# hby1320/pytorch_object_detection

Hardware: AMD Instinct MI355X
Metric: images/sec HISFCOS-R50 640x640 inference (higher is better)
Workload: dtype f32

## Files before the change

### include/fcosdet.h

```cpp
#ifndef FCOSDET_H_
#define FCOSDET_H_

#include <stdint.h>

#ifdef __cplusplus
extern "C" {
#endif

#define FD_OK 0
#define FD_E_INVAL (-1)
#define FD_E_UNSUPPORTED (-2)
#define FD_E_LAUNCH (-3)

#define FD_MAX_SEG 8

#define FD_ACT_NONE 0
#define FD_ACT_RELU 1
#define FD_ACT_SILU 2
#define FD_ACT_EXP 3
#define FD_ACT_SIGMOID 4

typedef void* fd_stream_t;

typedef struct fd_segs {
// ... 33 lines not shown
#define FD_TILE_WINOGRAD4 16
#define FD_TILE_NARROW 17
#define FD_TILE_F16K64 18
#define FD_TILE_COUNT 19

typedef struct fd_conv_params {
    const float* x;
    const float* w;
    const float* scale;
    const float* shift;
    const float* res;
    float* y;
    int32_t x_cs, x_co;
    int32_t res_cs, res_co;
    int32_t y_cs, y_co;
    int32_t Cin, Cout, KH, KW, stride, pad, dil;
    int32_t act;
    int32_t act_c0;
    int32_t mode;
    int32_t tile;
    int32_t tag;
    int32_t ksplit;
    void* workspace;
    int64_t workspace_bytes;
    int32_t precision;
    int32_t res_mode;
    float seg_param[FD_MAX_SEG];
    fd_segs in;
    int32_t out_H, out_W;
    int32_t sc_sy, sc_sx, sc_oy, sc_ox, sc_H, sc_W;
    const float* gate;
    int32_t gate_cs;
    int32_t reserved0;
    const float* w_frag;
    float* gn_stats;
    int32_t gn_groups;
    int32_t gate_act;
    const float* gate_b;
    const float* x2;
    int32_t x2_cs, x2_co, x2_Cin, x2_stride, x2_H, x2_W;
    int32_t wg_first, wg_count;
    int32_t sk_wgs;
    int32_t io_f16;
} fd_conv_params;
int64_t fd_conv_sk_workspace_bytes(int32_t sk_wgs);

int32_t fd_conv2d_nhwc_f32(const fd_conv_params* p, fd_stream_t stream);
int32_t fd_conv_workgroups(const fd_conv_params* p);
int32_t fd_conv_workgroups_live(const fd_conv_params* p);
typedef struct fd_b2b_params {
    const float* x; const float* w1_frag; const float* scale1; const float* shift1; const float* res; float* y;
    const float* w2_frag; const float* scale2; const float* shift2; float* z;
    int32_t x_cs, x_co, res_cs, res_co, y_cs, y_co, z_cs, z_co;
    int32_t K1, N1, N2, act1, act2, reserved0;
    int64_t rows;
} fd_b2b_params;
int32_t fd_conv1x1_b2b_f32(const fd_b2b_params* p, fd_stream_t stream);
int32_t fd_conv_narrow_nco(int32_t Cout);
int64_t fd_conv_workspace_bytes(int64_t out_rows, int32_t Cout, int32_t ksplit);

int64_t fd_wino4_weight_bytes(int32_t N, int32_t K);
int32_t fd_wino4_pack_weights_f32(const float* w, const float* scale, float* out, int32_t Cout, int32_t Cin, int32_t mode, fd_stream_t stream);

int64_t fd_conv_weight_wave_bytes(int32_t Cout, int32_t Cin);
int32_t fd_pack_conv_weight_wave_f32(const float* w, float* out, int32_t Cout, int32_t Cin, fd_stream_t stream);

int64_t fd_wino_weight_bytes(int32_t Cout, int32_t Cin);
int32_t fd_wino_pack_weights_f32(const float* w, const float* scale, float* out, int32_t Cout, int32_t Cin, int32_t mode,
                                 fd_stream_t stream);

typedef struct fd_conv_wgrad_params {
    const float* x;
    const float* dy;
    float* dw;
    int32_t x_cs, x_co, dy_cs, dy_co;
    int32_t Cin, Cout, KH, KW, stride, pad, dil;
    void* workspace;
    int64_t workspace_bytes;
    int32_t nsplit;
    int32_t layout;
    const float* scale;
    fd_segs in;
    int32_t precision;
    int32_t io_f16;
} fd_conv_wgrad_params;

int64_t fd_conv_wgrad_workspace_bytes(int64_t out_rows, int32_t Cin, int32_t Cout, int32_t KH, int32_t KW);
int32_t fd_conv2d_bwd_weight_f32(const fd_conv_wgrad_params* p, fd_stream_t stream);
int32_t fd_pack_conv_weight_f32(const float* w, const float* scale, float* out, int32_t Cout, int32_t Cin, int32_t KH,
                                int32_t KW, int32_t mode, fd_stream_t stream);

typedef struct fd_pack_job {
    const float* w;
    const float* scale;
    float* out;
    int32_t Cout, Cin, KH, KW, mode, reserved;
} fd_pack_job;
int32_t fd_pack_conv_weights_batch_f32(const fd_pack_job* jobs_dev, int32_t n_jobs, int64_t max_elems, fd_stream_t stream);

int32_t fd_stem7x7_nhwc4(const float* x4, const float* w, const float* scale, const float* shift, float* y, int32_t y_cs, int32_t y_co,
                         int32_t N, int32_t H, int32_t W, int32_t act, fd_stream_t stream);

int32_t fd_stem7x7_pool_nhwc4(const float* x4, const float* w, const float* scale, const float* shift, float* y_pooled, int32_t y_cs, int32_t y_co,
                              int32_t N, int32_t H, int32_t W, fd_stream_t stream);

int32_t fd_stem7x7_nchw3(const float* x, const float* w, const float* scale, const float* shift, float* y, int32_t y_cs, int32_t y_co,
                         int32_t N, int32_t H, int32_t W, int32_t act, int32_t pool, fd_stream_t stream);

// ... 214 lines not shown
```

### pytorch_object_detection_amd/_lib.py

```python
from __future__ import annotations

import ctypes as C
import os

FD_MAX_SEG = 8
ACT_NONE, ACT_RELU, ACT_SILU, ACT_EXP, ACT_SIGMOID = 0, 1, 2, 3, 4
CONV_GENERIC, CONV_STEM = 0, 1
PREC_F32, PREC_F16X3, PREC_F16 = 0, 1, 2
TILES = {1: (128, 128), 2: (128, 64), 3: (64, 128), 4: (64, 64), 5: (128, 32), 6: (128, 96),
         7: (128, 128), 8: (128, 64), 9: (64, 128),
         10: (256, 128), 11: (256, 128),
         12: (128, 96),
         13: (128, 128),
         15: (64, 64)}
PATCH_TILE = 13
WAVE_TILE = 15
WINO_TILE = 14
WINO4_TILE = 16
NARROW_TILE = 17
F16K64_TILE = 18

_HERE = os.path.dirname(os.path.abspath(__file__))
LIB_PATH = os.environ.get("FD_LIB") or os.path.join(_HERE, "csrc", "libfcosdet_hip.so")


class FdError(RuntimeError):

    def __init__(self, msg: str = "", rc=None):
        super().__init__(msg)
        self.rc = rc


E_INVAL, E_UNSUPPORTED, E_LAUNCH = -1, -2, -3


class Segs(C.Structure):
    _fields_ = [("nseg", C.c_int32), ("batch", C.c_int32), ("H", C.c_int32 * FD_MAX_SEG), ("W", C.c_int32 * FD_MAX_SEG),
                ("m_start", C.c_int32 * (FD_MAX_SEG + 1))]

    @staticmethod
    def make(batch: int, hw) -> "Segs":
        s = Segs()
        s.nseg, s.batch = len(hw), batch
        m = 0
        for i, (h, w) in enumerate(hw):
            s.H[i], s.W[i], s.m_start[i] = h, w, m
            m += batch * h * w
        for i in range(len(hw), FD_MAX_SEG + 1):
            s.m_start[i] = m
        return s

    @property
    def rows(self) -> int:
        return self.m_start[self.nseg]

    def level_hw(self):
        return [(self.H[i], self.W[i]) for i in range(self.nseg)]


class B2BParams(C.Structure):
    _fields_ = [("x", C.c_void_p), ("w1_frag", C.c_void_p), ("scale1", C.c_void_p), ("shift1", C.c_void_p), ("res", C.c_void_p), ("y", C.c_void_p),
                ("w2_frag", C.c_void_p), ("scale2", C.c_void_p), ("shift2", C.c_void_p), ("z", C.c_void_p),
                ("x_cs", C.c_int32), ("x_co", C.c_int32), ("res_cs", C.c_int32), ("res_co", C.c_int32), ("y_cs", C.c_int32), ("y_co", C.c_int32),
                ("z_cs", C.c_int32), ("z_co", C.c_int32),
                ("K1", C.c_int32), ("N1", C.c_int32), ("N2", C.c_int32), ("act1", C.c_int32), ("act2", C.c_int32), ("reserved0", C.c_int32),
                ("rows", C.c_int64)]


class ConvParams(C.Structure):
    _fields_ = [("x", C.c_void_p), ("w", C.c_void_p), ("scale", C.c_void_p), ("shift", C.c_void_p), ("res", C.c_void_p),
                ("y", C.c_void_p),
                ("x_cs", C.c_int32), ("x_co", C.c_int32), ("res_cs", C.c_int32), ("res_co", C.c_int32),
                ("y_cs", C.c_int32), ("y_co", C.c_int32),
                ("Cin", C.c_int32), ("Cout", C.c_int32), ("KH", C.c_int32), ("KW", C.c_int32), ("stride", C.c_int32),
                ("pad", C.c_int32), ("dil", C.c_int32),
                ("act", C.c_int32), ("act_c0", C.c_int32), ("mode", C.c_int32), ("tile", C.c_int32), ("tag", C.c_int32), ("ksplit", C.c_int32),
                ("workspace", C.c_void_p), ("workspace_bytes", C.c_int64), ("precision", C.c_int32), ("res_mode", C.c_int32),
                ("seg_param", C.c_float * FD_MAX_SEG), ("segs", Segs),
                ("out_H", C.c_int32), ("out_W", C.c_int32), ("sc_sy", C.c_int32), ("sc_sx", C.c_int32), ("sc_oy", C.c_int32),
                ("sc_ox", C.c_int32), ("sc_H", C.c_int32), ("sc_W", C.c_int32),
                ("gate", C.c_void_p), ("gate_cs", C.c_int32), ("reserved0", C.c_int32), ("w_frag", C.c_void_p),
                ("gn_stats", C.c_void_p), ("gn_groups", C.c_int32), ("gate_act", C.c_int32), ("gate_b", C.c_void_p),
                ("x2", C.c_void_p), ("x2_cs", C.c_int32), ("x2_co", C.c_int32), ("x2_Cin", C.c_int32), ("x2_stride", C.c_int32), ("x2_H", C.c_int32),
                ("x2_W", C.c_int32), ("wg_first", C.c_int32), ("wg_count", C.c_int32), ("sk_wgs", C.c_int32), ("io_f16", C.c_int32)]


class PackJob(C.Structure):
    _fields_ = [("w", C.c_void_p), ("scale", C.c_void_p), ("out", C.c_void_p), ("Cout", C.c_int32), ("Cin", C.c_int32),
                ("KH", C.c_int32), ("KW", C.c_int32), ("mode", C.c_int32), ("reserved", C.c_int32)]


class WgradParams(C.Structure):
    _fields_ = [("x", C.c_void_p), ("dy", C.c_void_p), ("dw", C.c_void_p),
                ("x_cs", C.c_int32), ("x_co", C.c_int32), ("dy_cs", C.c_int32), ("dy_co", C.c_int32),
                ("Cin", C.c_int32), ("Cout", C.c_int32), ("KH", C.c_int32), ("KW", C.c_int32), ("stride", C.c_int32),
                ("pad", C.c_int32), ("dil", C.c_int32),
                ("workspace", C.c_void_p), ("workspace_bytes", C.c_int64), ("nsplit", C.c_int32), ("layout", C.c_int32),
                ("scale", C.c_void_p), ("segs", Segs), ("precision", C.c_int32), ("io_f16", C.c_int32)]


_lib = None

_P, _I, _F, _D, _L = C.c_void_p, C.c_int32, C.c_float, C.c_double, C.c_int64
_SIGS = {
    "fd_version": (_I, []),
    "fd_last_error": (C.c_char_p, []),
    "fd_conv2d_nhwc_f32": (_I, [C.POINTER(ConvParams), _P]),
    "fd_conv_narrow_nco": (_I, [_I]),
    "fd_conv_workgroups": (_I, [C.POINTER(ConvParams)]),
    "fd_conv_workgroups_live": (_I, [C.POINTER(ConvParams)]),
    "fd_conv1x1_b2b_f32": (_I, [C.POINTER(B2BParams), _P]),
    "fd_conv_workspace_bytes": (_L, [_L, _I, _I]),
    "fd_conv_sk_workspace_bytes": (_L, [_I]),
    "fd_mbconv_pool_bytes": (_L, [_I, _I, _I, _I, _I, _I]),
    "fd_mbconv_expand_dw_nhwc": (_I, [_P, _I, _I, _P, _P, _P, _P, _P, _P, _P, _I, _I, _P, _I, _I, _I, _I, _I, _I, _I, _I, _I, _I, _I, _P]),
    "fd_se_gate_from_pool": (_I, [_P, _I, _P, _P, _P, _P, _I, _I, _I, _I, _P, _P]),
    "fd_conv_wgrad_workspace_bytes": (_L, [_L, _I, _I, _I, _I]),
    "fd_pack_conv_weight_f32": (_I, [_P, _P, _P, _I, _I, _I, _I, _I, _P]),
    "fd_pack_conv_weights_batch_f32": (_I, [_P, _I, _L, _P]),
# ... 100 lines not shown
```

### pytorch_object_detection_amd/csrc/fd_conv_b2b.hip

```cpp
#include "fd_conv_common.h"

struct B2BArgs {
    const float* x; const float* res; float* y; float* z;
    const float* scale1; const float* shift1; const float* scale2; const float* shift2;
    int x_cs, x_co, res_cs, res_co, y_cs, y_co, z_cs, z_co;
    int M, KT1, NT1, N2, act1, act2;
    unsigned x_bytes, y_bytes, z_bytes, res_bytes;
};

template <int TM, int TN2>
__global__ __launch_bounds__(64, 2) void conv1x1_b2b_kernel(B2BArgs a, const float* __restrict__ wf1_, const float* __restrict__ wf2_) {
    extern __shared__ __attribute__((aligned(16))) char smem[];
    float* As = reinterpret_cast<float*>(smem);
    float* A2 = As + 32 * TM * 32;
    constexpr int NL = 4 * TM;
    const int lane = threadIdx.x, l31 = lane & 31, lh = lane >> 5;
    const int m0 = blockIdx.x * 32 * TM;

    constexpr unsigned OOB = 0xC0000000u;
    const __amdgpu_buffer_rsrc_t xrsrc = __builtin_amdgcn_make_buffer_rsrc((void*)a.x, (short)0, (int)a.x_bytes, 0x00020000);
    const int lrow = lane >> 3, chunk = lane & 7;
    unsigned a_off[NL];
#pragma unroll
    for (int i = 0; i < NL; ++i) {
        const int m = m0 + lrow + 8 * i;
        a_off[i] = (m < a.M) ? ((unsigned)m * (unsigned)a.x_cs + (unsigned)(a.x_co + chunk * 4)) * 4u : OOB;
    }
    const float4* __restrict__ wf1 = reinterpret_cast<const float4*>(wf1_) + lane;
    const float4* __restrict__ wf2 = reinterpret_cast<const float4*>(wf2_) + lane;
    const int KT1 = a.KT1, KT2 = 2 * a.NT1;

    float4 ra[NL];
    auto load_a = [&](int kt) {
        const unsigned kb = (unsigned)kt * 128u;
#pragma unroll
        for (int i = 0; i < NL; ++i)
            ra[i] = __builtin_bit_cast(float4, __builtin_amdgcn_raw_buffer_load_b128(xrsrc, (int)(a_off[i] + kb), 0, 0));
    };
    auto store_a = [&]() {
#pragma unroll
        for (int i = 0; i < NL; ++i) *reinterpret_cast<float4*>(As + lds_off(lrow + 8 * i, chunk)) = ra[i];
    };

    f32x16 acc2[TM][TN2];
#pragma unroll
    for (int i = 0; i < TM; ++i)
#pragma unroll
        for (int j = 0; j < TN2; ++j)
#pragma unroll
            for (int e = 0; e < 16; ++e) acc2[i][j][e] = 0.f;

    const int c4 = (lane & 7) * 4, prow = lane >> 3;
    float* stage = As;
    const __amdgpu_buffer_rsrc_t yrsrc = __builtin_amdgcn_make_buffer_rsrc((void*)a.y, (short)0, (int)a.y_bytes, 0x00020000);
    const __amdgpu_buffer_rsrc_t zrsrc = __builtin_amdgcn_make_buffer_rsrc((void*)a.z, (short)0, (int)a.z_bytes, 0x00020000);
    const __amdgpu_buffer_rsrc_t rrsrc = __builtin_amdgcn_make_buffer_rsrc((void*)(a.res ? a.res : a.x), (short)0, (int)a.res_bytes, 0x00020000);
    const unsigned y_off = ((unsigned)(m0 + prow) * (unsigned)a.y_cs + (unsigned)(a.y_co + c4)) * 4u;
    const unsigned z_off = ((unsigned)(m0 + prow) * (unsigned)a.z_cs + (unsigned)(a.z_co + c4)) * 4u;
    const unsigned r_off = ((unsigned)(m0 + prow) * (unsigned)a.res_cs + (unsigned)(a.res_co + c4)) * 4u;

    for (int n1t = 0; n1t < a.NT1; ++n1t) {
        f32x16 acc1[TM][2];
#pragma unroll
        for (int i = 0; i < TM; ++i)
#pragma unroll
            for (int j = 0; j < 2; ++j)
#pragma unroll
                for (int e = 0; e < 16; ++e) acc1[i][j][e] = 0.f;
        float4 fb[2][2];
        const float4* __restrict__ w1t = wf1 + (size_t)n1t * KT1 * 512;
        load_a(0);
#pragma unroll
        for (int j = 0; j < 2; ++j)
#pragma unroll
            for (int s = 0; s < 2; ++s) fb[j][s] = w1t[(j * 4 + s) * 64];
        for (int kt = 0; kt < KT1; ++kt) {
            store_a();
            __builtin_amdgcn_sched_barrier(0);
            if (kt + 1 < KT1) load_a(kt + 1);
            __builtin_amdgcn_sched_barrier(0);
            wave_lds_sync();
            const float4* __restrict__ wc_ = w1t + (size_t)kt * 512;
            const float4* __restrict__ wn_ = w1t + (size_t)min(kt + 1, KT1 - 1) * 512;
            __builtin_amdgcn_s_setprio(1);
#pragma unroll
            for (int s = 0; s < 4; ++s) {
                float4 fa[TM];
#pragma unroll
                for (int i = 0; i < TM; ++i) fa[i] = *reinterpret_cast<const float4*>(As + lds_off(i * 32 + l31, 2 * s + lh));
#pragma unroll
                for (int i = 0; i < TM; ++i)
#pragma unroll
                    for (int j = 0; j < 2; ++j) {
                        acc1[i][j] = __builtin_amdgcn_mfma_f32_32x32x2f32(fa[i].x, fb[j][s & 1].x, acc1[i][j], 0, 0, 0);
                        acc1[i][j] = __builtin_amdgcn_mfma_f32_32x32x2f32(fa[i].y, fb[j][s & 1].y, acc1[i][j], 0, 0, 0);
                        acc1[i][j] = __builtin_amdgcn_mfma_f32_32x32x2f32(fa[i].z, fb[j][s & 1].z, acc1[i][j], 0, 0, 0);
                        acc1[i][j] = __builtin_amdgcn_mfma_f32_32x32x2f32(fa[i].w, fb[j][s & 1].w, acc1[i][j], 0, 0, 0);
                    }
#pragma unroll
                for (int j = 0; j < 2; ++j) fb[j][s & 1] = s < 2 ? wc_[(j * 4 + s + 2) * 64] : wn_[(j * 4 + s - 2) * 64];
                __builtin_amdgcn_sched_barrier(0);
            }
            __builtin_amdgcn_s_setprio(0);
            wave_lds_sync();
        }

#pragma unroll
        for (int j = 0; j < 2; ++j) {
            const int nb = n1t * 64 + 32 * j;
            const float sc = a.scale1 ? a.scale1[nb + l31] : 1.0f, sf = a.shift1 ? a.shift1[nb + l31] : 0.0f;
            float4 fb2[TN2][2];
            const int kt2 = 2 * n1t + j;
            auto w2at = [&](int jj, int s) { return wf2[((size_t)((jj >> 1) * KT2 + kt2) * 8 + (jj & 1) * 4 + s) * 64]; };
#pragma unroll
            for (int jj = 0; jj < TN2; ++jj)
#pragma unroll
                for (int s = 0; s < 2; ++s) fb2[jj][s] = w2at(jj, s);
#pragma unroll
            for (int i = 0; i < TM; ++i) {
                float4 rr[4];
#pragma unroll
                for (int p = 0; p < 4; ++p)
                    rr[p] = __builtin_bit_cast(float4, __builtin_amdgcn_raw_buffer_load_b128(rrsrc, (int)r_off, ((32 * i + 8 * p) * a.res_cs + nb) * 4, 0));
#pragma unroll
                for (int e = 0; e < 16; ++e) stage[((e & 3) + 8 * (e >> 2) + 4 * lh) * 32 + l31] = acc1[i][j][e] * sc + sf;
                wave_lds_sync();
#pragma unroll
                for (int p = 0; p < 4; ++p) {
                    float4 v = *reinterpret_cast<const float4*>(stage + (prow + 8 * p) * 32 + c4);
                    const float4 r = rr[p];
                    v.x += r.x; v.y += r.y; v.z += r.z; v.w += r.w;
                    if (a.act1 == FD_ACT_RELU) {
                        v.x = fmaxf(v.x, 0.f); v.y = fmaxf(v.y, 0.f); v.z = fmaxf(v.z, 0.f); v.w = fmaxf(v.w, 0.f);
                    } else if (a.act1 == FD_ACT_SILU) {
                        v.x = fd_act(v.x, FD_ACT_SILU, 0.f); v.y = fd_act(v.y, FD_ACT_SILU, 0.f); v.z = fd_act(v.z, FD_ACT_SILU, 0.f); v.w = fd_act(v.w, FD_ACT_SILU, 0.f);
                    }
                    __builtin_amdgcn_raw_buffer_store_b128(__builtin_bit_cast(f32x4, v), yrsrc, (int)y_off, ((32 * i + 8 * p) * a.y_cs + nb) * 4, 0);
                    *reinterpret_cast<float4*>(A2 + lds_off(32 * i + prow + 8 * p, lane & 7)) = v;
                }
                wave_lds_sync();
            }
            __builtin_amdgcn_s_setprio(1);
#pragma unroll
            for (int s = 0; s < 4; ++s) {
                float4 fa[TM];
#pragma unroll
                for (int i = 0; i < TM; ++i) fa[i] = *reinterpret_cast<const float4*>(A2 + lds_off(i * 32 + l31, 2 * s + lh));
#pragma unroll
                for (int i = 0; i < TM; ++i)
#pragma unroll
                    for (int jj = 0; jj < TN2; ++jj) {
                        acc2[i][jj] = __builtin_amdgcn_mfma_f32_32x32x2f32(fa[i].x, fb2[jj][s & 1].x, acc2[i][jj], 0, 0, 0);
                        acc2[i][jj] = __builtin_amdgcn_mfma_f32_32x32x2f32(fa[i].y, fb2[jj][s & 1].y, acc2[i][jj], 0, 0, 0);
                        acc2[i][jj] = __builtin_amdgcn_mfma_f32_32x32x2f32(fa[i].z, fb2[jj][s & 1].z, acc2[i][jj], 0, 0, 0);
                        acc2[i][jj] = __builtin_amdgcn_mfma_f32_32x32x2f32(fa[i].w, fb2[jj][s & 1].w, acc2[i][jj], 0, 0, 0);
                    }
                if (s < 2) {
#pragma unroll
                    for (int jj = 0; jj < TN2; ++jj) fb2[jj][s & 1] = w2at(jj, s + 2);
                }
                __builtin_amdgcn_sched_barrier(0);
            }
            __builtin_amdgcn_s_setprio(0);
            wave_lds_sync();
        }
    }

#pragma unroll
    for (int jj = 0; jj < TN2; ++jj) {
        const int nb = 32 * jj;
        if (nb >= a.N2) break;
        const float sc = a.scale2 ? a.scale2[nb + l31] : 1.0f, sf = a.shift2 ? a.shift2[nb + l31] : 0.0f;
#pragma unroll
        for (int i = 0; i < TM; ++i) {
#pragma unroll
            for (int e = 0; e < 16; ++e) stage[((e & 3) + 8 * (e >> 2) + 4 * lh) * 32 + l31] = acc2[i][jj][e] * sc + sf;
            wave_lds_sync();
#pragma unroll
            for (int p = 0; p < 4; ++p) {
                float4 v = *reinterpret_cast<const float4*>(stage + (prow + 8 * p) * 32 + c4);
                if (a.act2 == FD_ACT_RELU) {
                    v.x = fmaxf(v.x, 0.f); v.y = fmaxf(v.y, 0.f); v.z = fmaxf(v.z, 0.f); v.w = fmaxf(v.w, 0.f);
                } else if (a.act2 == FD_ACT_SILU) {
                    v.x = fd_act(v.x, FD_ACT_SILU, 0.f); v.y = fd_act(v.y, FD_ACT_SILU, 0.f); v.z = fd_act(v.z, FD_ACT_SILU, 0.f); v.w = fd_act(v.w, FD_ACT_SILU, 0.f);
                }
                __builtin_amdgcn_raw_buffer_store_b128(__builtin_bit_cast(f32x4, v), zrsrc, (int)z_off, ((32 * i + 8 * p) * a.z_cs + nb) * 4, 0);
            }
            wave_lds_sync();
        }
    }
}

extern "C" int32_t fd_conv1x1_b2b_f32(const fd_b2b_params* p, fd_stream_t stream_) {
    hipStream_t stream = (hipStream_t)stream_;
    FD_REQUIRE(p && p->x && p->w1_frag && p->w2_frag && p->y && p->z, FD_E_INVAL, "fd_conv1x1_b2b: null pointer");
    FD_REQUIRE(p->rows >= 1 && p->K1 >= 32 && p->K1 % 32 == 0 && p->N1 >= 64 && p->N1 % 64 == 0 && (p->N2 == 64 || p->N2 == 128), FD_E_UNSUPPORTED,
               "fd_conv1x1_b2b: needs K1 %% 32 == 0, N1 %% 64 == 0, N2 in {64, 128} (got %d -> %d -> %d)", p->K1, p->N1, p->N2);
    FD_REQUIRE(p->x_cs % 4 == 0 && p->x_co % 4 == 0 && p->x_cs >= p->x_co + p->K1 && p->y_cs % 4 == 0 && p->y_co % 4 == 0 && p->y_cs >= p->y_co + p->N1 &&
                   p->z_cs % 4 == 0 && p->z_co % 4 == 0 && p->z_cs >= p->z_co + p->N2 &&
                   (!p->res || (p->res_cs % 4 == 0 && p->res_co % 4 == 0 && p->res_cs >= p->res_co + p->N1)),
               FD_E_INVAL, "fd_conv1x1_b2b: channel views must be 4-aligned and in range");
    FD_REQUIRE((((uintptr_t)p->x | (uintptr_t)p->y | (uintptr_t)p->z | (uintptr_t)p->res | (uintptr_t)p->w1_frag | (uintptr_t)p->w2_frag) & 15) == 0, FD_E_INVAL,
               "fd_conv1x1_b2b: pointers must be 16-byte aligned");
    auto act_ok = [](int a_) { return a_ == FD_ACT_NONE || a_ == FD_ACT_RELU || a_ == FD_ACT_SILU; };
    FD_REQUIRE(act_ok(p->act1) && act_ok(p->act2), FD_E_UNSUPPORTED, "fd_conv1x1_b2b: activations none / ReLU / SiLU");
    const long xb = (long)p->rows * p->x_cs * 4;
    FD_REQUIRE(xb < 0xC0000000L - 65536 && (long)p->rows * p->y_cs * 4 < 0xC0000000L && (long)p->rows * p->z_cs * 4 < 0xC0000000L &&
                   (!p->res || (long)p->rows * p->res_cs * 4 < 0xC0000000L), FD_E_UNSUPPORTED, "fd_conv1x1_b2b: a view's buffer exceeds 3 GiB");
    B2BArgs a;
    a.x = p->x; a.res = p->res; a.y = p->y; a.z = p->z;
    a.scale1 = p->scale1; a.shift1 = p->shift1; a.scale2 = p->scale2; a.shift2 = p->shift2;
    a.x_cs = p->x_cs; a.x_co = p->x_co; a.res_cs = p->res_cs; a.res_co = p->res_co; a.y_cs = p->y_cs; a.y_co = p->y_co; a.z_cs = p->z_cs; a.z_co = p->z_co;
    a.M = (int)p->rows; a.KT1 = p->K1 / 32; a.NT1 = p->N1 / 64; a.N2 = p->N2; a.act1 = p->act1; a.act2 = p->act2;
    a.x_bytes = (unsigned)xb;
    a.y_bytes = (unsigned)((long)p->rows * p->y_cs * 4); a.z_bytes = (unsigned)((long)p->rows * p->z_cs * 4);
    a.res_bytes = p->res ? (unsigned)((long)p->rows * p->res_cs * 4) : 0u;
    if (p->N2 == 64) {
        const unsigned blocks = (unsigned)((p->rows + 63) / 64);
        hipLaunchKernelGGL((conv1x1_b2b_kernel<2, 2>), dim3(blocks), dim3(64), 2 * 64 * 32 * 4, stream, a, p->w1_frag, p->w2_frag);
    } else {
        const unsigned blocks = (unsigned)((p->rows + 31) / 32);
        hipLaunchKernelGGL((conv1x1_b2b_kernel<1, 4>), dim3(blocks), dim3(64), 2 * 32 * 32 * 4, stream, a, p->w1_frag, p->w2_frag);
    }
    FD_CHECK_LAUNCH("fd_conv1x1_b2b_f32");
    return FD_OK;
}
```

### pytorch_object_detection_amd/engine.py

```python
from __future__ import annotations

from typing import Callable, Dict, List, Optional, Sequence, Tuple

import torch

from . import ops
from . import _lib
from ._lib import ACT_EXP, ACT_NONE, ACT_RELU, ACT_SILU, FdError, Segs
from .ops import Rows


import os as _os

CONV_PRECISION = _os.environ.get("FD_CONV_PRECISION", "f32")
AUTOTUNE = True
GN_FUSED = _os.environ.get("FD_GN_FUSED", "1") != "0"
B2B_MIN_ROWS = 64 * 1024
B2B_LAYERS = "1"


class PRows(Rows):
    __slots__ = ("_flat",)


class Pool:

    def __init__(self, device):
        self.device = device
        self.free: List[torch.Tensor] = []
        self.total = 0

    def get(self, rows: int, C: int) -> PRows:
        need = rows * C
        best = None
        for i, t in enumerate(self.free):
            if t.numel() >= need and (best is None or t.numel() < self.free[best].numel()):
                best = i
        if best is None:
            flat = torch.empty(need, dtype=torch.float32, device=self.device)
            self.total += need * 4
        else:
            flat = self.free.pop(best)
        r = PRows(flat[:need].view(rows, C))
        r._flat = flat
        return r

    def put(self, r: PRows) -> None:
        self.free.append(r._flat)


class Plan:
    def __init__(self, device, precision: Optional[str] = None, pair_tuned: bool = False):
        self.device = device
        self.steps: List[Callable[[], None]] = []
        self.names: List[str] = []
        self.pool = Pool(device)
        self.keep: List[object] = []
        self.flops = 0
        self.step_flops: Dict[int, int] = {}
        self.step_info: Dict[int, dict] = {}
        self.marks: Dict[str, Tuple[int, int]] = {}
        self.autotune = AUTOTUNE
        self.precision = precision or CONV_PRECISION
        if self.precision not in ("f32", "f16x3", "mixed"):
            raise FdError(f"unknown conv precision '{self.precision}' (f32 | f16x3 | mixed)")
        self.tiles: Dict[str, int] = {}
        self.pair_tuned = pair_tuned

    def add(self, name: str, fn: Callable[[], None]) -> None:
        self.steps.append(fn)
        self.names.append(name)
# ... 211 lines not shown
    else:
        plan.add("input.nchw3_to_nhwc4", lambda: ops.nchw3_to_nhwc4(image_ref[0], x4.buf))


def build_resnet50(plan: Plan, trunk, batch: int, H: int, W: int, image_ref: List[torch.Tensor]):
    dev, pool = plan.device, plan.pool
    stem_own = plan.precision in ("f32", "mixed") and tuple(trunk.conv1.weight.shape) == (64, 3, 7, 7)
    mode = getattr(plan, "input_mode", None) or ("u8" if getattr(plan, "input_u8", None) else None)
    nchw_in = stem_own and mode is None
    x4 = None
    if not nchw_in:
        x4 = pool.get(batch * H * W, 4)
        add_input(plan, x4, batch, H, W, image_ref)
    s_in = Segs.make(batch, [(H, W)])
    sc, sf = ops.fold_bn(_dev(trunk.bn1.weight, dev), _dev(trunk.bn1.bias, dev), _dev(trunk.bn1.running_mean, dev),
                         _dev(trunk.bn1.running_var, dev), trunk.bn1.eps)
    s1 = ops.conv_out_segs(s_in, 7, 2, 3, 1)
    H1, W1 = s1.H[0], s1.W[0]
    H2, W2 = (H1 + 2 - 3) // 2 + 1, (W1 + 2 - 3) // 2 + 1
    s2 = Segs.make(batch, [(H2, W2)])

    def nchw_image() -> torch.Tensor:
        x = image_ref[0]
        if tuple(x.shape) != (batch, 3, H, W):
            raise FdError(f"plan input: expected a [{batch}, 3, {H}, {W}] batch, got {tuple(x.shape)}")
        return x

    y1 = None
    if stem_own:
        wp = ops.pack_stem7_weight(_dev(trunk.conv1.weight, dev))
        y2 = pool.get(s2.rows, 64)
        if nchw_in:
            plan.add("backbone.conv1+maxpool", lambda: ops.stem7x7_nchw(nchw_image(), wp, y2, sc, sf, pool=True))
        else:
            plan.add("backbone.conv1+maxpool", lambda: ops.stem7x7_pool(x4, wp, y2, batch, H, W, sc, sf))
    else:
        wp = ops.pack_stem_weight(_dev(trunk.conv1.weight, dev))
        y1 = pool.get(s1.rows, 64)
        plan.add("backbone.conv1", ops.conv_call(x4, s_in, wp, y1, Cin=4, Cout=64, k=7, stride=2, pad=3, scale=sc, shift=sf,
                                                 act=ACT_RELU, stem=True))
    plan.keep += [wp, sc, sf]
    plan.flops += 2 * s1.rows * 64 * 147
    plan.step_flops[len(plan.steps) - 1] = 2 * s1.rows * 64 * 147
    if x4 is not None:
        pool.put(x4)
    if y1 is not None:
        y2 = pool.get(s2.rows, 64)
        plan.add("backbone.maxpool", lambda: ops.maxpool(y1, y2, batch, H1, W1, 3, 2, 1))
        pool.put(y1)
    x, sx = y2, s2
    feats = []
    blocks_all = [(li, bi, blk) for li in (1, 2, 3, 4) for bi, blk in enumerate(getattr(trunk, f"layer{li}"))]
    o1_ready = None
    for gi, (li, bi, blk) in enumerate(blocks_all):
        nm = f"backbone.layer{li}.{bi}"
        planes = blk.conv1.weight.shape[0]
        so = ops.conv_out_segs(sx, 3, blk.conv2.stride[0], 1, 1)
        ds = blk.downsample
        if o1_ready is not None:
            o1, o1_ready = o1_ready, None
        else:
            o1 = pool.get(sx.rows, planes)
            add_conv(plan, nm + ".conv1", x, sx, blk.conv1, o1, bn=blk.bn1, act=ACT_RELU)
        o2 = pool.get(so.rows, planes)
        add_conv(plan, nm + ".conv2", o1, sx, blk.conv2, o2, bn=blk.bn2, act=ACT_RELU)
        pool.put(o1)
        dual = (ds is not None and plan.precision == "f32" and ds[0].kernel_size[0] == 1 and ds[0].bias is None and blk.conv3.bias is None
                and planes % 32 == 0 and x.C % 32 == 0 and x.cs % 4 == 0 and x.co % 4 == 0 and ds[0].stride[0] == blk.conv2.stride[0])
        if dual:
            f3 = ops.fold_bn(_dev(blk.bn3.weight, dev), _dev(blk.bn3.bias, dev), _dev(blk.bn3.running_mean, dev), _dev(blk.bn3.running_var, dev), blk.bn3.eps)
            fdn = ops.fold_bn(_dev(ds[1].weight, dev), _dev(ds[1].bias, dev), _dev(ds[1].running_mean, dev), _dev(ds[1].running_var, dev), ds[1].eps)
            wcat = torch.cat([_dev(blk.conv3.weight, dev) * f3[0][:, None, None, None], _dev(ds[0].weight, dev) * fdn[0][:, None, None, None]], 1)
            out = pool.get(so.rows, 4 * planes)
            add_conv(plan, nm + ".conv3+downsample", o2, so, blk.conv3, out, weight=wcat, fold=(None, (f3[1] + fdn[1]).contiguous()), act=ACT_RELU,
                     x2=x, x2_stride=ds[0].stride[0], x2_hw=(sx.H[0], sx.W[0]))
            plan.step_info[len(plan.steps) - 1]["dual"] = (planes, x.C, ds[0].stride[0])
            pool.put(o2)
            if not (feats and feats[-1][0] is x):
                pool.put(x)
            x, sx = out, so
            if li >= 2 and bi == len(getattr(trunk, f"layer{li}")) - 1:
                feats.append((x, sx))
            continue
        if ds is not None:
            idt = pool.get(so.rows, 4 * planes)
            add_conv(plan, nm + ".downsample", x, sx, ds[0], idt, bn=ds[1])
        else:
            idt = x
        out = pool.get(so.rows, 4 * planes)
        nxt = blocks_all[gi + 1][2] if gi + 1 < len(blocks_all) else None
        n2 = nxt.conv1.weight.shape[0] if nxt is not None else 0
        if (str(li) in B2B_LAYERS and so.rows >= B2B_MIN_ROWS and nxt is not None and plan.precision == "f32" and blk.conv3.bias is None and nxt.conv1.bias is None
                and nxt.conv1.kernel_size[0] == 1 and nxt.conv1.stride[0] == 1 and nxt.conv1.weight.shape[1] == 4 * planes
                and ops.b2b_ok(planes, 4 * planes, n2) and all(r.cs % 4 == 0 and r.co % 4 == 0 for r in (o2, out, idt))):
            o1_ready = pool.get(so.rows, n2)
            f3 = ops.fold_bn(_dev(blk.bn3.weight, dev), _dev(blk.bn3.bias, dev), _dev(blk.bn3.running_mean, dev), _dev(blk.bn3.running_var, dev), blk.bn3.eps)
            fn1 = ops.fold_bn(_dev(nxt.bn1.weight, dev), _dev(nxt.bn1.bias, dev), _dev(nxt.bn1.running_mean, dev), _dev(nxt.bn1.running_var, dev), nxt.bn1.eps)
            wa = ops.pack_conv_weight_wave(_dev(blk.conv3.weight, dev))
            wb = ops.pack_conv_weight_wave(_dev(nxt.conv1.weight, dev))
            plan.keep += [f3, fn1, wa, wb]
            nl, nb_ = blocks_all[gi + 1][0], blocks_all[gi + 1][1]
            plan.add(f"{nm}.conv3+layer{nl}.{nb_}.conv1",
                     ops.conv_b2b_call(o2, wa, out, wb, o1_ready, K1=planes, N1=4 * planes, N2=n2, scale1=f3[0], shift1=f3[1], res=idt, act1=ACT_RELU,
                                       scale2=fn1[0], shift2=fn1[1], act2=ACT_RELU))
            fl = 2 * so.rows * (4 * planes * planes + n2 * 4 * planes)
            plan.flops += fl
            plan.step_flops[len(plan.steps) - 1] = fl
            plan.step_info[len(plan.steps) - 1] = {"k": 1, "stride": 1, "dil": 1, "Cin": planes, "Cout": 4 * planes, "rows": so.rows, "family": "1x1",
                                                   "mfma_div": 1.0, "b2b": (4 * planes, n2)}
        else:
            add_conv(plan, nm + ".conv3", o2, so, blk.conv3, out, bn=blk.bn3, act=ACT_RELU, res=idt)
        pool.put(o2)
        if idt is not x:
            pool.put(idt)
        if not (feats and feats[-1][0] is x):
            pool.put(x)
        x, sx = out, so
        if li >= 2 and bi == len(getattr(trunk, f"layer{li}")) - 1:
            feats.append((x, sx))
    return feats


def build_efficientnet(plan: Plan, net, batch: int, H: int, W: int, image_ref: List[torch.Tensor], keep=(2, 3, 4)):
    dev, pool = plan.device, plan.pool
    x4 = pool.get(batch * H * W, 4)
    add_input(plan, x4, batch, H, W, image_ref)

    def out_hw(h: int, w: int, k: int, s: int, pad) -> Tuple[int, int]:
        return (h + pad[0] + pad[1] - k) // s + 1, (w + pad[0] + pad[1] - k) // s + 1

    def bn_fold(bn):
        sc, sf = ops.fold_bn(_dev(bn.weight, dev), _dev(bn.bias, dev), _dev(bn.running_mean, dev), _dev(bn.running_var, dev), bn.eps)
        plan.keep += [sc, sf]
        return sc, sf

    stem = net._conv_stem
    C0 = stem.weight.shape[0]
    h, w = out_hw(H, W, 3, 2, net.stem_pad)
    ws = ops.pack_stem3_weight(_dev(stem.weight, dev))
    sc0, sf0 = bn_fold(net._bn0)
    plan.keep.append(ws)
    x = pool.get(batch * h * w, C0)
    plan.add("backbone._conv_stem", lambda x=x, h=h, w=w: ops.stem_conv3(x4.buf, ws, x, batch, H, W, 3, 2, net.stem_pad[0], net.stem_pad[0],
                                                                       h, w, sc0, sf0, ACT_SILU))
    plan.flops += 2 * batch * h * w * C0 * 27
    pool.put(x4)
    blocks = list(net._blocks)
    ends: List[Optional[Tuple[Rows, Segs]]] = []
    for bi, blk in enumerate(blocks):
        nm = f"backbone._blocks.{bi}"
        segs = Segs.make(batch, [(h, w)])
        inp = x
        mid = blk._depthwise_conv.weight.shape[0]
        ho, wo = out_hw(h, w, blk.kernel, blk.stride, blk.pad)
        if ho < 1 or wo < 1:
            raise FdError("EfficientNet: input too small")
        so = Segs.make(batch, [(ho, wo)])
        fused = (blk.expand != 1 and plan.precision == "f32" and blk._expand_conv.bias is None and not (blk.kernel == 5 and blk.stride == 2)
                 and ops.mbconv_fused_ok(x.C, mid, blk.kernel, blk.stride) and x.C == blk._expand_conv.weight.shape[1])
        d = pool.get(so.rows, mid)
        wd = ops.pack_dwk_weight(_dev(blk._depthwise_conv.weight, dev))
        sc, sf = bn_fold(blk._bn1)
        pool_part = None
# ... 495 lines not shown
```

### pytorch_object_detection_amd/ops.py

```python
from __future__ import annotations

import ctypes as C
import enum
import json
import math
import os
import re
from typing import Callable, List, NamedTuple, Optional, Sequence, Tuple

import numpy as np
import torch

from . import _lib
from ._lib import ACT_EXP, ACT_NONE, ACT_RELU, ACT_SIGMOID, ACT_SILU, ConvParams, FdError, Segs, check


CONV_LOG = None
LAUNCHES = [0]


def _stream() -> int:
    LAUNCHES[0] += 1
    return torch.cuda.current_stream().cuda_stream

# ... 258 lines not shown
    if not W4_SK:
        return 0
    table = _tune_table()
    if _TUNE_MODE != "force" and key in table:
        return int(table[key])
    if _TUNE_MODE == "0":
        return 0
    best, best_t = 0, float("inf")
    for wgs in (0, 256, 240):
        call = conv_sk(run, wgs, ws) if wgs else run
        try:
            call()
        except FdError as e:
            if e.rc != _lib.E_UNSUPPORTED:
                raise
            continue
        t = min(_time_launches(call, reps, False) for _ in range(3))
        if t < best_t * 0.98:
            best, best_t = wgs, t
    table[key] = best
    return best


def conv_workgroups(run) -> Tuple[int, int]:
    n = _lib.lib().fd_conv_workgroups(C.byref(run.params))
    live = _lib.lib().fd_conv_workgroups_live(C.byref(run.params))
    if n < 0 or live < 0:
        raise FdError("fd_conv_workgroups: " + _lib.lib().fd_last_error().decode(errors="replace"), int(min(n, live)))
    return (run.params.wg_count or n), live


def conv_wg_slice(run, first: int, count: int, tag: Optional[int] = None) -> Callable[[], None]:
    q = _lib.ConvParams()
    C.memmove(C.byref(q), C.byref(run.params), C.sizeof(q))
    q.wg_first, q.wg_count = first, count
    if tag is not None:
        q.tag = tag
    fn = _lib.lib().fd_conv2d_nhwc_f32
    ref = C.byref(q)

    def run_slice(_keep=(run, q)):
        check(fn(ref, _stream()), "fd_conv2d_nhwc_f32")

    run_slice.params = q
    return run_slice


def b2b_ok(K1: int, N1: int, N2: int) -> bool:
    return K1 % 32 == 0 and N1 % 64 == 0 and N2 in (64, 128)


def conv_b2b_call(x: Rows, w1_frag: torch.Tensor, y: Rows, w2_frag: torch.Tensor, z: Rows, *, K1: int, N1: int, N2: int,
                  scale1: Optional[torch.Tensor] = None, shift1: Optional[torch.Tensor] = None, res: Optional[Rows] = None, act1: int = ACT_NONE,
                  scale2: Optional[torch.Tensor] = None, shift2: Optional[torch.Tensor] = None, act2: int = ACT_NONE) -> Callable[[], None]:
    _need_gpu(w1_frag, w2_frag, scale1, shift1, scale2, shift2)
    p = _lib.B2BParams()
    p.x, p.w1_frag, p.y, p.w2_frag, p.z = x.ptr, w1_frag.data_ptr(), y.ptr, w2_frag.data_ptr(), z.ptr
    p.scale1 = scale1.data_ptr() if scale1 is not None else None
    p.shift1 = shift1.data_ptr() if shift1 is not None else None
    p.scale2 = scale2.data_ptr() if scale2 is not None else None
    p.shift2 = shift2.data_ptr() if shift2 is not None else None
    p.res = res.ptr if res is not None else None
    p.x_cs, p.x_co, p.y_cs, p.y_co, p.z_cs, p.z_co = x.cs, x.co, y.cs, y.co, z.cs, z.co
    if res is not None:
        p.res_cs, p.res_co = res.cs, res.co
    p.K1, p.N1, p.N2, p.act1, p.act2, p.rows = K1, N1, N2, act1, act2, y.rows
    fn = _lib.lib().fd_conv1x1_b2b_f32
    ref = C.byref(p)
    keep = (x, w1_frag, y, w2_frag, z, scale1, shift1, scale2, shift2, res, p)

    def run(_keep=keep):
        check(fn(ref, _stream()), "fd_conv1x1_b2b_f32")

    run.params = p
    return run


_TUNE_CACHE: dict = {}
_TUNE_FILE = os.environ.get("FD_TILE_TABLE") or os.path.join(os.path.dirname(os.path.abspath(__file__)), "tuned", "gfx950_tiles.json")
_TUNE_MODE = os.environ.get("FD_AUTOTUNE", "0")
_TUNE_LOADED = False


def _tune_table() -> dict:
    global _TUNE_LOADED
    if not _TUNE_LOADED:
        _TUNE_LOADED = True
        try:
            with open(_TUNE_FILE) as f:
                _TUNE_CACHE.update(json.load(f))
        except Exception:
            pass
    return _TUNE_CACHE


def save_tune_table() -> None:
    os.makedirs(os.path.dirname(_TUNE_FILE), exist_ok=True)
    with open(_TUNE_FILE, "w") as f:
        json.dump(dict(sorted(_TUNE_CACHE.items())), f, indent=0)


KSPLIT_MAX = 8
_BKEY = re.compile(r"^(f16x3\|)?B(\d+)(\|.*)$")


def tile_code(tile: int, ksplit: int = 1) -> int:
    return tile | ((ksplit if ksplit > 1 else 0) << 8)


def tile_split(code: int) -> Tuple[int, int]:
    return code & 0xFF, max(1, code >> 8)


def tune_key(segs: Segs, Cin: int, Cout: int, k: int = 3, stride: int = 1, pad: int = 1, dil: int = 1, *, res: bool = False, xcs: int = 0,
             ycs: int = 0, pre: str = "", x2: Optional[Tuple[int, int]] = None, rup: bool = False) -> str:
    hw = "+".join(f"{h}x{w}" for h, w in segs.level_hw())
    if pre == "w4sk":
        return f"w4sk|B{segs.batch}|{hw}|{Cin}>{Cout}|d{dil}|res{int(res)}"
    key = f"B{segs.batch}|{hw}|{Cin}>{Cout}|k{k}s{stride}p{pad}d{dil}|res{int(res)}|xcs{xcs}|ycs{ycs}"
# ... 1186 lines not shown
```

Measured before the change: 1434.

## Write only stride-2 subsampled rows of b2b conv3 output feeding next downsample

```diff
diff --git a/include/fcosdet.h b/include/fcosdet.h
--- a/include/fcosdet.h
+++ b/include/fcosdet.h
@@ -109,8 +109,10 @@
     const float* x; const float* w1_frag; const float* scale1; const float* shift1; const float* res; float* y;
     const float* w2_frag; const float* scale2; const float* shift2; float* z;
     int32_t x_cs, x_co, res_cs, res_co, y_cs, y_co, z_cs, z_co;
-    int32_t K1, N1, N2, act1, act2, reserved0;
+    int32_t K1, N1, N2, act1, act2, y_sub;
     int64_t rows;
+    int64_t y_rows;
+    int32_t y_batch, y_H, y_W, reserved0;
 } fd_b2b_params;
 int32_t fd_conv1x1_b2b_f32(const fd_b2b_params* p, fd_stream_t stream);
 int32_t fd_conv_narrow_nco(int32_t Cout);
diff --git a/pytorch_object_detection_amd/_lib.py b/pytorch_object_detection_amd/_lib.py
--- a/pytorch_object_detection_amd/_lib.py
+++ b/pytorch_object_detection_amd/_lib.py
@@ -63,8 +63,8 @@
                 ("w2_frag", C.c_void_p), ("scale2", C.c_void_p), ("shift2", C.c_void_p), ("z", C.c_void_p),
                 ("x_cs", C.c_int32), ("x_co", C.c_int32), ("res_cs", C.c_int32), ("res_co", C.c_int32), ("y_cs", C.c_int32), ("y_co", C.c_int32),
                 ("z_cs", C.c_int32), ("z_co", C.c_int32),
-                ("K1", C.c_int32), ("N1", C.c_int32), ("N2", C.c_int32), ("act1", C.c_int32), ("act2", C.c_int32), ("reserved0", C.c_int32),
-                ("rows", C.c_int64)]
+                ("K1", C.c_int32), ("N1", C.c_int32), ("N2", C.c_int32), ("act1", C.c_int32), ("act2", C.c_int32), ("y_sub", C.c_int32),
+                ("rows", C.c_int64), ("y_rows", C.c_int64), ("y_batch", C.c_int32), ("y_H", C.c_int32), ("y_W", C.c_int32), ("reserved0", C.c_int32)]
 
 
 class ConvParams(C.Structure):
diff --git a/pytorch_object_detection_amd/csrc/fd_conv_b2b.hip b/pytorch_object_detection_amd/csrc/fd_conv_b2b.hip
--- a/pytorch_object_detection_amd/csrc/fd_conv_b2b.hip
+++ b/pytorch_object_detection_amd/csrc/fd_conv_b2b.hip
@@ -5,10 +5,11 @@
     const float* scale1; const float* shift1; const float* scale2; const float* shift2;
     int x_cs, x_co, res_cs, res_co, y_cs, y_co, z_cs, z_co;
     int M, KT1, NT1, N2, act1, act2;
+    int H, W, H2, W2;
     unsigned x_bytes, y_bytes, z_bytes, res_bytes;
 };
 
-template <int TM, int TN2>
+template <int TM, int TN2, bool SUB>
 __global__ __launch_bounds__(64, 2) void conv1x1_b2b_kernel(B2BArgs a, const float* __restrict__ wf1_, const float* __restrict__ wf2_) {
     extern __shared__ __attribute__((aligned(16))) char smem[];
     float* As = reinterpret_cast<float*>(smem);
@@ -58,6 +59,17 @@
     const unsigned y_off = ((unsigned)(m0 + prow) * (unsigned)a.y_cs + (unsigned)(a.y_co + c4)) * 4u;
     const unsigned z_off = ((unsigned)(m0 + prow) * (unsigned)a.z_cs + (unsigned)(a.z_co + c4)) * 4u;
     const unsigned r_off = ((unsigned)(m0 + prow) * (unsigned)a.res_cs + (unsigned)(a.res_co + c4)) * 4u;
+    unsigned ys_row = 0, ys_lane = 0;
+    unsigned long long live = 0;
+    if constexpr (SUB) {
+        const unsigned m = (unsigned)m0 + (unsigned)(lane & (32 * TM - 1));
+        const unsigned q = m / (unsigned)a.W, w = m - q * (unsigned)a.W;
+        const unsigned n = q / (unsigned)a.H, h = q - n * (unsigned)a.H;
+        const bool on = m < (unsigned)a.M && ((h | w) & 1u) == 0;
+        ys_row = on ? ((n * (unsigned)a.H2 + (h >> 1)) * (unsigned)a.W2 + (w >> 1)) * (unsigned)a.y_cs * 4u : OOB;
+        ys_lane = (unsigned)(a.y_co + c4) * 4u;
+        live = __builtin_amdgcn_ballot_w64(on);
+    }
 
     for (int n1t = 0; n1t < a.NT1; ++n1t) {
         f32x16 acc1[TM][2];
@@ -135,7 +147,14 @@
                     } else if (a.act1 == FD_ACT_SILU) {
                         v.x = fd_act(v.x, FD_ACT_SILU, 0.f); v.y = fd_act(v.y, FD_ACT_SILU, 0.f); v.z = fd_act(v.z, FD_ACT_SILU, 0.f); v.w = fd_act(v.w, FD_ACT_SILU, 0.f);
                     }
-                    __builtin_amdgcn_raw_buffer_store_b128(__builtin_bit_cast(f32x4, v), yrsrc, (int)y_off, ((32 * i + 8 * p) * a.y_cs + nb) * 4, 0);
+                    if constexpr (SUB) {
+                        if ((unsigned)(live >> (8 * (4 * i + p))) & 0xFFu) {
+                            const unsigned o = (unsigned)__builtin_amdgcn_ds_bpermute((prow + 8 * (4 * i + p)) * 4, (int)ys_row) + ys_lane;
+                            __builtin_amdgcn_raw_buffer_store_b128(__builtin_bit_cast(f32x4, v), yrsrc, (int)o, nb * 4, 0);
+                        }
+                    } else {
+                        __builtin_amdgcn_raw_buffer_store_b128(__builtin_bit_cast(f32x4, v), yrsrc, (int)y_off, ((32 * i + 8 * p) * a.y_cs + nb) * 4, 0);
+                    }
                     *reinterpret_cast<float4*>(A2 + lds_off(32 * i + prow + 8 * p, lane & 7)) = v;
                 }
                 wave_lds_sync();
@@ -204,23 +223,37 @@
                "fd_conv1x1_b2b: pointers must be 16-byte aligned");
     auto act_ok = [](int a_) { return a_ == FD_ACT_NONE || a_ == FD_ACT_RELU || a_ == FD_ACT_SILU; };
     FD_REQUIRE(act_ok(p->act1) && act_ok(p->act2), FD_E_UNSUPPORTED, "fd_conv1x1_b2b: activations none / ReLU / SiLU");
+    const int sub = p->y_sub == 0 ? 1 : p->y_sub;
+    FD_REQUIRE(sub == 1 || sub == 2, FD_E_UNSUPPORTED, "fd_conv1x1_b2b: y_sub must be 1 or 2 (got %d)", p->y_sub);
+    long y_rows = p->rows;
+    if (sub == 2) {
+        FD_REQUIRE(p->y_batch >= 1 && p->y_H >= 1 && p->y_W >= 1 && (long)p->y_batch * p->y_H * p->y_W == p->rows, FD_E_UNSUPPORTED,
+                   "fd_conv1x1_b2b: y_sub = 2 needs the map geometry, batch * H * W == rows (got %d x %d x %d, %ld rows)", p->y_batch, p->y_H, p->y_W, (long)p->rows);
+        y_rows = (long)p->y_batch * ((p->y_H + 1) / 2) * ((p->y_W + 1) / 2);
+        FD_REQUIRE(p->y_rows >= y_rows, FD_E_UNSUPPORTED, "fd_conv1x1_b2b: the compact y view holds %ld rows, y_sub = 2 writes %ld", (long)p->y_rows, y_rows);
+    }
     const long xb = (long)p->rows * p->x_cs * 4;
-    FD_REQUIRE(xb < 0xC0000000L - 65536 && (long)p->rows * p->y_cs * 4 < 0xC0000000L && (long)p->rows * p->z_cs * 4 < 0xC0000000L &&
+    FD_REQUIRE(xb < 0xC0000000L - 65536 && y_rows * p->y_cs * 4 < 0xC0000000L && (long)p->rows * p->z_cs * 4 < 0xC0000000L &&
                    (!p->res || (long)p->rows * p->res_cs * 4 < 0xC0000000L), FD_E_UNSUPPORTED, "fd_conv1x1_b2b: a view's buffer exceeds 3 GiB");
     B2BArgs a;
     a.x = p->x; a.res = p->res; a.y = p->y; a.z = p->z;
     a.scale1 = p->scale1; a.shift1 = p->shift1; a.scale2 = p->scale2; a.shift2 = p->shift2;
     a.x_cs = p->x_cs; a.x_co = p->x_co; a.res_cs = p->res_cs; a.res_co = p->res_co; a.y_cs = p->y_cs; a.y_co = p->y_co; a.z_cs = p->z_cs; a.z_co = p->z_co;
     a.M = (int)p->rows; a.KT1 = p->K1 / 32; a.NT1 = p->N1 / 64; a.N2 = p->N2; a.act1 = p->act1; a.act2 = p->act2;
+    a.H = sub == 2 ? p->y_H : 1; a.W = sub == 2 ? p->y_W : 1; a.H2 = (a.H + 1) / 2; a.W2 = (a.W + 1) / 2;
     a.x_bytes = (unsigned)xb;
-    a.y_bytes = (unsigned)((long)p->rows * p->y_cs * 4); a.z_bytes = (unsigned)((long)p->rows * p->z_cs * 4);
+    a.y_bytes = (unsigned)(y_rows * p->y_cs * 4); a.z_bytes = (unsigned)((long)p->rows * p->z_cs * 4);
     a.res_bytes = p->res ? (unsigned)((long)p->rows * p->res_cs * 4) : 0u;
-    if (p->N2 == 64) {
+    if (p->N2 == 64 && sub == 2) {
+        const unsigned blocks = (unsigned)((p->rows + 31) / 32);
+        hipLaunchKernelGGL((conv1x1_b2b_kernel<1, 2, true>), dim3(blocks), dim3(64), 2 * 32 * 32 * 4, stream, a, p->w1_frag, p->w2_frag);
+    } else if (p->N2 == 64) {
         const unsigned blocks = (unsigned)((p->rows + 63) / 64);
-        hipLaunchKernelGGL((conv1x1_b2b_kernel<2, 2>), dim3(blocks), dim3(64), 2 * 64 * 32 * 4, stream, a, p->w1_frag, p->w2_frag);
+        hipLaunchKernelGGL((conv1x1_b2b_kernel<2, 2, false>), dim3(blocks), dim3(64), 2 * 64 * 32 * 4, stream, a, p->w1_frag, p->w2_frag);
     } else {
         const unsigned blocks = (unsigned)((p->rows + 31) / 32);
-        hipLaunchKernelGGL((conv1x1_b2b_kernel<1, 4>), dim3(blocks), dim3(64), 2 * 32 * 32 * 4, stream, a, p->w1_frag, p->w2_frag);
+        if (sub == 2) hipLaunchKernelGGL((conv1x1_b2b_kernel<1, 4, true>), dim3(blocks), dim3(64), 2 * 32 * 32 * 4, stream, a, p->w1_frag, p->w2_frag);
+        else hipLaunchKernelGGL((conv1x1_b2b_kernel<1, 4, false>), dim3(blocks), dim3(64), 2 * 32 * 32 * 4, stream, a, p->w1_frag, p->w2_frag);
     }
     FD_CHECK_LAUNCH("fd_conv1x1_b2b_f32");
     return FD_OK;
diff --git a/pytorch_object_detection_amd/engine.py b/pytorch_object_detection_amd/engine.py
--- a/pytorch_object_detection_amd/engine.py
+++ b/pytorch_object_detection_amd/engine.py
@@ -17,6 +17,7 @@
 GN_FUSED = _os.environ.get("FD_GN_FUSED", "1") != "0"
 B2B_MIN_ROWS = 64 * 1024
 B2B_LAYERS = "1"
+B2B_Y_SUBSAMPLE = True
 
 
 class PRows(Rows):
@@ -334,6 +335,13 @@
     feats = []
     blocks_all = [(li, bi, blk) for li in (1, 2, 3, 4) for bi, blk in enumerate(getattr(trunk, f"layer{li}"))]
     o1_ready = None
+    x_sub = False
+
+    def dual_ok(blk, xC: int, xcs: int, xco: int) -> bool:
+        ds, planes = blk.downsample, blk.conv1.weight.shape[0]
+        return (ds is not None and plan.precision == "f32" and ds[0].kernel_size[0] == 1 and ds[0].bias is None and blk.conv3.bias is None
+                and planes % 32 == 0 and xC % 32 == 0 and xcs % 4 == 0 and xco % 4 == 0 and ds[0].stride[0] == blk.conv2.stride[0])
+
     for gi, (li, bi, blk) in enumerate(blocks_all):
         nm = f"backbone.layer{li}.{bi}"
         planes = blk.conv1.weight.shape[0]
@@ -347,15 +355,17 @@
         o2 = pool.get(so.rows, planes)
         add_conv(plan, nm + ".conv2", o1, sx, blk.conv2, o2, bn=blk.bn2, act=ACT_RELU)
         pool.put(o1)
-        dual = (ds is not None and plan.precision == "f32" and ds[0].kernel_size[0] == 1 and ds[0].bias is None and blk.conv3.bias is None
-                and planes % 32 == 0 and x.C % 32 == 0 and x.cs % 4 == 0 and x.co % 4 == 0 and ds[0].stride[0] == blk.conv2.stride[0])
+        dual = dual_ok(blk, x.C, x.cs, x.co)
+        if x_sub and not dual:
+            raise FdError(f"{nm}: the block's input was written subsampled for a conv3 + downsample launch the block does not take")
         if dual:
             f3 = ops.fold_bn(_dev(blk.bn3.weight, dev), _dev(blk.bn3.bias, dev), _dev(blk.bn3.running_mean, dev), _dev(blk.bn3.running_var, dev), blk.bn3.eps)
             fdn = ops.fold_bn(_dev(ds[1].weight, dev), _dev(ds[1].bias, dev), _dev(ds[1].running_mean, dev), _dev(ds[1].running_var, dev), ds[1].eps)
             wcat = torch.cat([_dev(blk.conv3.weight, dev) * f3[0][:, None, None, None], _dev(ds[0].weight, dev) * fdn[0][:, None, None, None]], 1)
             out = pool.get(so.rows, 4 * planes)
             add_conv(plan, nm + ".conv3+downsample", o2, so, blk.conv3, out, weight=wcat, fold=(None, (f3[1] + fdn[1]).contiguous()), act=ACT_RELU,
-                     x2=x, x2_stride=ds[0].stride[0], x2_hw=(sx.H[0], sx.W[0]))
+                     x2=x, x2_stride=1 if x_sub else ds[0].stride[0], x2_hw=(so.H[0], so.W[0]) if x_sub else (sx.H[0], sx.W[0]))
+            x_sub = False
             plan.step_info[len(plan.steps) - 1]["dual"] = (planes, x.C, ds[0].stride[0])
             pool.put(o2)
             if not (feats and feats[-1][0] is x):
@@ -369,12 +379,16 @@
             add_conv(plan, nm + ".downsample", x, sx, ds[0], idt, bn=ds[1])
         else:
             idt = x
-        out = pool.get(so.rows, 4 * planes)
         nxt = blocks_all[gi + 1][2] if gi + 1 < len(blocks_all) else None
         n2 = nxt.conv1.weight.shape[0] if nxt is not None else 0
         if (str(li) in B2B_LAYERS and so.rows >= B2B_MIN_ROWS and nxt is not None and plan.precision == "f32" and blk.conv3.bias is None and nxt.conv1.bias is None
                 and nxt.conv1.kernel_size[0] == 1 and nxt.conv1.stride[0] == 1 and nxt.conv1.weight.shape[1] == 4 * planes
-                and ops.b2b_ok(planes, 4 * planes, n2) and all(r.cs % 4 == 0 and r.co % 4 == 0 for r in (o2, out, idt))):
+                and ops.b2b_ok(planes, 4 * planes, n2) and all(r.cs % 4 == 0 and r.co % 4 == 0 for r in (o2, idt))):
+            last = bi == len(getattr(trunk, f"layer{li}")) - 1
+            x_sub = (B2B_Y_SUBSAMPLE and last and li < 2 and nxt.conv2.stride[0] == 2 and so.nseg == 1
+                     and dual_ok(nxt, 4 * planes, 4 * planes, 0))
+            sub_hw = ((so.H[0] + 1) // 2, (so.W[0] + 1) // 2)
+            out = pool.get(batch * sub_hw[0] * sub_hw[1] if x_sub else so.rows, 4 * planes)
             o1_ready = pool.get(so.rows, n2)
             f3 = ops.fold_bn(_dev(blk.bn3.weight, dev), _dev(blk.bn3.bias, dev), _dev(blk.bn3.running_mean, dev), _dev(blk.bn3.running_var, dev), blk.bn3.eps)
             fn1 = ops.fold_bn(_dev(nxt.bn1.weight, dev), _dev(nxt.bn1.bias, dev), _dev(nxt.bn1.running_mean, dev), _dev(nxt.bn1.running_var, dev), nxt.bn1.eps)
@@ -384,13 +398,15 @@
             nl, nb_ = blocks_all[gi + 1][0], blocks_all[gi + 1][1]
             plan.add(f"{nm}.conv3+layer{nl}.{nb_}.conv1",
                      ops.conv_b2b_call(o2, wa, out, wb, o1_ready, K1=planes, N1=4 * planes, N2=n2, scale1=f3[0], shift1=f3[1], res=idt, act1=ACT_RELU,
-                                       scale2=fn1[0], shift2=fn1[1], act2=ACT_RELU))
+                                       scale2=fn1[0], shift2=fn1[1], act2=ACT_RELU, y_sub=2 if x_sub else 1,
+                                       y_geom=(batch, so.H[0], so.W[0]) if x_sub else None))
             fl = 2 * so.rows * (4 * planes * planes + n2 * 4 * planes)
             plan.flops += fl
             plan.step_flops[len(plan.steps) - 1] = fl
             plan.step_info[len(plan.steps) - 1] = {"k": 1, "stride": 1, "dil": 1, "Cin": planes, "Cout": 4 * planes, "rows": so.rows, "family": "1x1",
                                                    "mfma_div": 1.0, "b2b": (4 * planes, n2)}
         else:
+            out = pool.get(so.rows, 4 * planes)
             add_conv(plan, nm + ".conv3", o2, so, blk.conv3, out, bn=blk.bn3, act=ACT_RELU, res=idt)
         pool.put(o2)
         if idt is not x:
diff --git a/pytorch_object_detection_amd/ops.py b/pytorch_object_detection_amd/ops.py
--- a/pytorch_object_detection_amd/ops.py
+++ b/pytorch_object_detection_amd/ops.py
@@ -334,7 +334,8 @@
 
 def conv_b2b_call(x: Rows, w1_frag: torch.Tensor, y: Rows, w2_frag: torch.Tensor, z: Rows, *, K1: int, N1: int, N2: int,
                   scale1: Optional[torch.Tensor] = None, shift1: Optional[torch.Tensor] = None, res: Optional[Rows] = None, act1: int = ACT_NONE,
-                  scale2: Optional[torch.Tensor] = None, shift2: Optional[torch.Tensor] = None, act2: int = ACT_NONE) -> Callable[[], None]:
+                  scale2: Optional[torch.Tensor] = None, shift2: Optional[torch.Tensor] = None, act2: int = ACT_NONE,
+                  y_sub: int = 1, y_geom: Optional[Tuple[int, int, int]] = None) -> Callable[[], None]:
     _need_gpu(w1_frag, w2_frag, scale1, shift1, scale2, shift2)
     p = _lib.B2BParams()
     p.x, p.w1_frag, p.y, p.w2_frag, p.z = x.ptr, w1_frag.data_ptr(), y.ptr, w2_frag.data_ptr(), z.ptr
@@ -346,7 +347,10 @@
     p.x_cs, p.x_co, p.y_cs, p.y_co, p.z_cs, p.z_co = x.cs, x.co, y.cs, y.co, z.cs, z.co
     if res is not None:
         p.res_cs, p.res_co = res.cs, res.co
-    p.K1, p.N1, p.N2, p.act1, p.act2, p.rows = K1, N1, N2, act1, act2, y.rows
+    p.K1, p.N1, p.N2, p.act1, p.act2, p.rows = K1, N1, N2, act1, act2, z.rows
+    p.y_sub, p.y_rows = y_sub, y.rows
+    if y_geom is not None:
+        p.y_batch, p.y_H, p.y_W = y_geom
     fn = _lib.lib().fd_conv1x1_b2b_f32
     ref = C.byref(p)
     keep = (x, w1_frag, y, w2_frag, z, scale1, shift1, scale2, shift2, res, p)
```

New measurement: 1437, median of 6. No clear change (+0.3%).
